# pySTEPS/pysteps

Hardware: AMD Instinct MI355X
Metric: Mpixels*leadsteps/s (LK+semilag) at 4096x4096 fp32 (higher is better)
Workload: dtype f32

## Files before the change

pysteps_amd/csrc/common.h:

```cpp
#pragma once

#include <hip/hip_runtime.h>

#include <cmath>
#include <cstdarg>
#include <cstddef>
#include <cstdint>
#include <cstdio>
#include <mutex>

#include "../../include/pysteps_hip.h"
#include "entry.h"
#include "scratch.h"

#ifdef PSH_DEBUG
#include <cassert>
#define PSH_DASSERT(cond) assert(cond)
#else
#define PSH_DASSERT(cond) ((void)0)
#endif

namespace psh {

constexpr int kNumXcd = 8;
// ... 128 lines not shown
                                  int capacity, int k, double thr, unsigned char *flags_dev,
                                  hipStream_t stream);
int lk_track_pool(void *pyramid_handle, const float *points_host, const float *points_dev, const int *npts_dev,
                  int npts, int max_count, double epsilon, double min_eig_threshold, double *pool_xy_dev,
                  double *pool_uv_dev, int *pool_count_dev, int pool_capacity);

int lk_corners_resident(const unsigned char *feature_u8_dev, const float *clean_dev, float *stats_dev, int m, int n,
                        int block_size, int buffer_mask, double quality_level, double min_distance, int max_corners,
                        float *points_dev, int *npoints_dev, int (*before_walk)(void *) = nullptr,
                        void *before_walk_arg = nullptr, int *walk_stats_host = nullptr,
                        unsigned *slots_cleared = nullptr);

size_t lk_prepare_ws_bytes(int m, int n, bool f64);
int lk_prepare_on(hipStream_t stream, void *ws, const void *frame_dev, bool f64, int m, int n, int size_opening,
                  int buffer_mask, float *clean_dev, unsigned char *track_u8_dev, unsigned char *feature_u8_dev,
                  float *stats_dev, unsigned *slots_cleared = nullptr, unsigned long long *keepbits = nullptr);
size_t lk_keepbits_bytes(int m, int n);
size_t lk_slot_bytes();
int lk_pyramids_on_side(hipStream_t side, void *block, size_t block_bytes, const unsigned char *prev_u8_dev,
                        const unsigned char *next_u8_dev, int m, int n, int win_w, int win_h, int max_level,
                        void **handle_out);
size_t lk_pyramids_bytes(int m, int n, int win_w, int win_h, int max_level);

int corner_order_max_corners();
bool corner_order_supported(int m, int n, double min_distance, int max_corners);
size_t corner_order_ws_bytes();
hipError_t launch_corner_order(const unsigned long long *raw_dev, const int *raw_count_dev, int cap,
                               const float *eig_max_dev, float quality, int n, double min_distance,
                               int max_corners, void *ws_dev, float *points_dev, int *npoints_dev,
                               hipStream_t stream, int (*before_walk)(void *), void *before_walk_arg,
                               bool ws_is_cleared, const unsigned *eig_slots_dev = nullptr, int count_bias = 0,
                               float *eig_max_out_dev = nullptr);
size_t corner_order_clear_bytes();
size_t corner_order_walk_stats_offset();
hipError_t launch_vectors_finish(const double *pool_xy_dev, const double *pool_uv_dev,
                                 const unsigned char *flags_dev, const int *pool_count_dev, int capacity,
                                 double decl_scale, int m, int n, float *xy_out_dev, float *uv_out_dev,
                                 IdwDyn *dyn_dev, hipStream_t stream);

}
```

pysteps_amd/csrc/lk.hip:

```cpp
#include <algorithm>
#include <cmath>
#include <cstring>
#include <functional>
#include <vector>

#include "common.h"

#pragma clang fp contract(off)

namespace psh {
namespace {

enum Stat : int {
  kMinAll = 0,
  kNanCount,
  kMaxAll,
  kMinFeat,
  kMaxFeat,
  kEigMax,
  kNumStats = 8
};

constexpr int kRedBlocks = 1024;

// ... 619 lines not shown
  return true;
}

__device__ __forceinline__ float next_lane_f(float v) {
  return __int_as_float(__builtin_amdgcn_update_dpp(0, __float_as_int(v), 0x130 , 0xf, 0xf, true));
}
__device__ __forceinline__ double next_lane_d(double v) {
  const int lo = __builtin_amdgcn_update_dpp(0, __double2loint(v), 0x130, 0xf, 0xf, true);
  const int hi = __builtin_amdgcn_update_dpp(0, __double2hiint(v), 0x130, 0xf, 0xf, true);
  return __hiloint2double(hi, lo);
}
__device__ __forceinline__ bool walk_mirrored(int i, int n) {
  if (i >= 0 && i + 1 < n) return false;
  return reflect101(i + 1, n) != reflect101(reflect101(i, n) + 1, n);
}

constexpr int crn_cols(int block_size) { return 64 - 2 * (block_size / 2 + 1); }

template <int BS, int ROWS>
__global__ __launch_bounds__(256) void lk_corner_response_cols(
    const unsigned char *__restrict__ u8, const float *__restrict__ clean, int m, int n,
    int buffer_mask, const float *__restrict__ stats, float *__restrict__ eig,
    float *__restrict__ partial, Band band, unsigned *__restrict__ slots, int *__restrict__ zero_a, int count_a,
    int *__restrict__ zero_b, int count_b) {
  constexpr int r = BS / 2, H = r + 1, W = crn_cols(BS);
  if (blockIdx.x == 0 && blockIdx.y == 0) {
    for (int i = threadIdx.x; i < count_a; i += 256) zero_a[i] = 0;
    for (int i = threadIdx.x; i < count_b; i += 256) zero_b[i] = 0;
  }
  __shared__ float red[4];
  const int lane = threadIdx.x & 63, wave = __builtin_amdgcn_readfirstlane(threadIdx.x >> 6);
  const int x0 = blockIdx.x * W;
  const int yb = (blockIdx.y * 4 + wave) * ROWS;
  float best = 0.f;
  if (yb < m) {
    const float s = 1.0f / (4.0f * static_cast<float>(BS) * 255.0f), s2 = 2.f * s;
    const int xl = x0 - H + lane;
    const bool neg_x = walk_mirrored(xl + 1, n);
    const float sx = neg_x ? -s : s, sx2 = neg_x ? -s2 : s2;
    const unsigned char *col = u8 + reflect101(xl, n);
    const bool few_rows = m < 2 * H + 2;
    auto row_of = [&](int y) -> int {
      if (few_rows) return reflect101(y, m);
      y = y < 0 ? -y : y;
      return y >= m ? 2 * m - 2 - y : y;
    };
    auto load_row = [&](int i) -> int { return col[static_cast<size_t>(row_of(yb - H + i)) * n]; };
// ... 58 lines not shown
            t1 = next_lane_d(t1);
            t2 = next_lane_d(t2);
            w0 += t0;
            w1 += t1;
            w2 += t2;
          }
          const int y = yb + p - BS;
          if (writer) {
            const float a = static_cast<float>(w0) * 0.5f, b = static_cast<float>(w1);
            const float c = static_cast<float>(w2) * 0.5f;
            const float e = (a + c) - sqrtf((a - c) * (a - c) + b * b);
            eig[static_cast<size_t>(y) * n + x] = e;
            if (y >= band.lo && y < band.hi && px_allowed(clean, m, n, x, y, buffer_mask, any_nan))
              best = fmaxf(best, fmaxf(e, 0.f));
          }
        }
      }
#pragma unroll
      for (int j = 0; j < BS; ++j) raw[j] = nxt[j];
    }
  }
  best = wave_max(best);
  if (lane == 0) red[wave] = best;
  __syncthreads();
  if (threadIdx.x == 0) {
    const int b = blockIdx.y * gridDim.x + blockIdx.x;
    const float b_max = fmaxf(fmaxf(red[0], red[1]), fmaxf(red[2], red[3]));
    if (slots) {
      slot_max(slots, kSlEig, b, b_max);
    } else {
      partial[b] = b_max;
    }
  }
}

constexpr int kNmsKeys = 64;

using CornerKeyT = unsigned long long;
__device__ __forceinline__ CornerKeyT nms_key(float val, unsigned addr) {
  return (static_cast<CornerKeyT>(__float_as_uint(val)) << 32) | addr;
}
__device__ __forceinline__ float prev_lane_f(float v) {
  return __int_as_float(__builtin_amdgcn_update_dpp(0, __float_as_int(v), 0x138 , 0xf, 0xf, true));
}

template <int BS, int ROWS>
// ... 168 lines not shown

#ifndef PSH_SEL_WAVES
#define PSH_SEL_WAVES 4
#endif
#ifndef PSH_SEL_GROUPS
#define PSH_SEL_GROUPS 4
#endif
#ifndef PSH_SEL_WIDE
#define PSH_SEL_WIDE 1
#endif
constexpr int kSelWaves = PSH_SEL_WAVES;
constexpr int kSelGroups = PSH_SEL_GROUPS;
constexpr bool kSelWide = PSH_SEL_WIDE != 0;
constexpr int kSelCols = 62;
constexpr int kSelWgRows = kSelWide ? 16 * kSelGroups : 16 * kSelGroups * kSelWaves;
constexpr int kSelWgCols = kSelWide ? kSelCols * kSelWaves : kSelCols;

__global__ __launch_bounds__(64 * kSelWaves) void lk_corner_select(const float *__restrict__ eig,
                                                        const float *__restrict__ clean, int m,
                                                        int n, int buffer_mask, float quality,
                                                        float *__restrict__ stats,
                                                        CornerKey *__restrict__ out, int cap,
                                                        int *__restrict__ count, Band band,
                                                        const unsigned *__restrict__ slots) {
  constexpr int kRows = 16;
  __shared__ unsigned long long s_mask[kSelWaves][kSelGroups * kRows];
  __shared__ int wave_count[kSelWaves];
  __shared__ int block_base;
  const int lane = threadIdx.x & 63, wave = threadIdx.x >> 6;
  const int x = (kSelWide ? (blockIdx.x * kSelWaves + wave) : blockIdx.x) * kSelCols - 1 + lane, xc = x + 1;
  const int y_wave = (kSelWide ? blockIdx.y : (blockIdx.y * kSelWaves + wave)) * (kSelGroups * kRows);
  const float eig_max = slots ? slots_max(slots, kSlEig) : stats[kEigMax];
  if (slots && blockIdx.x == 0 && blockIdx.y == 0 && threadIdx.x == 0) stats[kEigMax] = eig_max;
  const float thr = eig_max * quality;
  const bool any_nan = stats[kNanCount] > 0.f;
  const bool col_in = x >= 0 && x < n;
  const bool col_ok = lane < kSelCols && xc >= 1 && xc < n - 1;
  int mine = 0;
  for (int g = 0; g < kSelGroups; ++g) {
    const int y_first = y_wave + g * kRows;
    if (y_first >= m) {
      if (lane < kRows) s_mask[wave][g * kRows + lane] = 0ull;
      continue;
    }
    float v[kRows + 2], m3[kRows + 2], hmax[kRows + 2];
#pragma unroll
    for (int q = 0; q < kRows + 2; ++q) {
      const int y = y_first - 1 + q;
      v[q] = (col_in && y >= 0 && y < m) ? eig[static_cast<size_t>(y) * n + x] : 0.f;
    }
#pragma unroll
    for (int q = 0; q < kRows + 2; ++q) {
      const float left = v[q], centre = next_lane_f(left), right = next_lane_f(centre);
      hmax[q] = fmaxf(left, right);
      m3[q] = fmaxf(centre, hmax[q]);
      v[q] = centre;
    }
#pragma unroll
    for (int r = 0; r < kRows; ++r) {
      const int yr = y_first + r;
      const float c = v[r + 1];
      bool keep = col_ok && yr >= 1 && yr < m - 1 && yr >= band.lo && yr < band.hi;
      keep = keep && c > thr && c != 0.f;
      keep = keep && !(fmaxf(hmax[r + 1], fmaxf(m3[r], m3[r + 2])) > c);
      keep = keep && px_allowed(clean, m, n, xc, yr, buffer_mask, any_nan);
      const unsigned long long mask = __ballot(keep);
      if (lane == 0) s_mask[wave][g * kRows + r] = mask;
      mine += __popcll(mask);
    }
  }
  if (lane == 0) wave_count[wave] = mine;
  __syncthreads();
  if (threadIdx.x == 0) {
    int total = 0;
    for (int w = 0; w < kSelWaves; ++w) total += wave_count[w];
    block_base = total > 0 ? atomicAdd(count, total) : 0;
  }
  __syncthreads();
  int pos = block_base;
  for (int w = 0; w < wave; ++w) pos += wave_count[w];
  if (mine == 0) return;
  for (int r = 0; r < kSelGroups * kRows; ++r) {
    const unsigned long long mask = s_mask[wave][r];
    if (mask == 0ull) continue;
    const int y = y_wave + r;
    if ((mask >> lane) & 1ull) {
      const int at = pos + __popcll(mask & ((1ull << lane) - 1ull));
      if (at < cap)
        out[at] = make_corner_key(eig[static_cast<size_t>(y) * n + xc], static_cast<unsigned>(y + band.y_org) * n + xc);
    }
    pos += __popcll(mask);
  }
}

constexpr int kPyrRows = 8;

struct PyrPair {
  const unsigned char *src[2];
  unsigned char *dst[2];
};

template <bool FAST>
__device__ __forceinline__ void pyr_rows(const unsigned char *__restrict__ src, unsigned char *__restrict__ dst, int m,
                                         int n, int om, int on, int ox, int oy0, int wx, const int (&off)[11]) {
  auto window = [&](const unsigned char *row) -> uint4 {
    if (FAST) return *reinterpret_cast<const uint4 *>(row + wx);
    unsigned w[4] = {0u, 0u, 0u, 0u};
#pragma unroll
    for (int k = 0; k < 11; ++k) w[(k + 2) >> 2] |= static_cast<unsigned>(row[off[k]]) << (8 * ((k + 2) & 3));
    return make_uint4(w[0], w[1], w[2], w[3]);
  };
  auto hrow = [&](const uint4 d, int h[4]) {
    const unsigned w[4] = {d.x, d.y, d.z, d.w};
    auto b = [&](int k) -> int { return static_cast<int>((w[(k + 2) >> 2] >> (8 * ((k + 2) & 3))) & 0xffu); };
// ... 564 lines not shown
  return dim3((n + w - 1) / w, (m + rows - 1) / rows);
}
int lk_response_nms_fixed_keys(dim3 grid) { return static_cast<int>(grid.x * grid.y) * 4 * kNmsKeys; }
void launch_lk_response_nms(dim3 grid, hipStream_t stream, int block_size, const unsigned char *u8, const float *clean, int m,
                            int n, int buffer_mask, const float *stats, float quality, CornerKeyT *out, int cap, Band band,
                            unsigned *slots, int *zero_b, int count_b) {
#define PSH_NMS_LAUNCH(BS)                                                                                             \
  hipLaunchKernelGGL((lk_corner_response_nms<BS, kCrnRows>), grid, dim3(256), 0, stream, u8, clean, m, n, buffer_mask, \
                     stats, quality, out, cap, band, slots, zero_b, count_b)
  if (block_size == 1) {
    PSH_NMS_LAUNCH(1);
  } else if (block_size == 3) {
    PSH_NMS_LAUNCH(3);
  } else if (block_size == 5) {
    PSH_NMS_LAUNCH(5);
  } else {
    PSH_NMS_LAUNCH(7);
  }
#undef PSH_NMS_LAUNCH
}
void launch_lk_response(dim3 grid, hipStream_t stream, int block_size, const unsigned char *u8, const float *clean, int m,
                        int n, int buffer_mask, const float *stats, float *eig, float *part, Band band,
                        unsigned *slots = nullptr, int *zero_a = nullptr, int count_a = 0, int *zero_b = nullptr,
                        int count_b = 0) {
#define PSH_CRN_LAUNCH(BS)                                                                                          \
  hipLaunchKernelGGL((lk_corner_response_cols<BS, kCrnRows>), grid, dim3(256), 0, stream, u8, clean, m, n, buffer_mask, \
                     stats, eig, part, band, slots, zero_a, count_a, zero_b, count_b)
  if (block_size == 1) {
    PSH_CRN_LAUNCH(1);
  } else if (block_size == 3) {
    PSH_CRN_LAUNCH(3);
  } else if (block_size == 5) {
    PSH_CRN_LAUNCH(5);
  } else {
    PSH_CRN_LAUNCH(7);
  }
#undef PSH_CRN_LAUNCH
}

static int ensure_lk_ws(size_t nbytes, void **ptr) {
  static void *ws = nullptr;
  const int rc = persistent_device(&ws, nbytes);
  *ptr = ws;
  return rc;
}

size_t lk_prepare_ws_bytes(int m, int n, bool f64) {
  const size_t npx = static_cast<size_t>(m) * n;
  if (f64) {
    const dim3 ogrid((n + kOpenColsW - 1) / kOpenColsW, (m + kOpenRowsWG - 1) / kOpenRowsWG);
// ... 133 lines not shown
  const float *img = frame_dev + static_cast<size_t>(e0) * n;
  float *clean = clean_dev + static_cast<size_t>(e0) * n;
  const psh::Band band{e0, r0 - e0, r1 - e0};
  psh::launch_lk_open(ogrid, c.stream, img, ms, n, size_opening, buffer_mask, stats_dev, clean, part, band);
  hipLaunchKernelGGL(psh::lk_open_final, dim3(1), dim3(psh::kFinalThreads), 0, c.stream, part, nb_open, stats_dev);
  PSH_HIP(hipGetLastError());
  return PSH_OK;
}

int psh_lk_band_to_u8_dev(const float *clean_dev, int m, int n, int e0, int e1, int buffer_mask, const float *stats_dev,
                          unsigned char *track_u8_dev, unsigned char *feature_u8_dev) {
  PSH_ENTER(c);
  if (!clean_dev || !stats_dev || !track_u8_dev) return fail(PSH_EINVAL, "lk_band_to_u8: NULL pointer");
  if (int rc = check_band("lk_band_to_u8", m, n, e0, e1, e0, e1)) return rc;
  const size_t off = static_cast<size_t>(e0) * n, npx = static_cast<size_t>(e1 - e0) * n;
  const int qgrid = static_cast<int>(std::min<size_t>((npx / 4 + 255) / 256 + 1, 4096));
  hipLaunchKernelGGL(psh::lk_to_u8, dim3(qgrid), dim3(256), 0, c.stream, clean_dev + off, e1 - e0, n, buffer_mask,
                     const_cast<float *>(stats_dev), track_u8_dev + off, feature_u8_dev ? feature_u8_dev + off : nullptr, e0,
                     static_cast<const unsigned *>(nullptr));
  PSH_HIP(hipGetLastError());
  return PSH_OK;
}

int psh_lk_band_response_dev(const unsigned char *feature_u8_dev, const float *clean_dev, int m, int n, int e0, int e1,
                             int r0, int r1, int block_size, int buffer_mask, float *stats_dev, float *eig_dev) {
  PSH_ENTER(c);
  if (!feature_u8_dev || !clean_dev || !stats_dev || !eig_dev) return fail(PSH_EINVAL, "lk_band_response: NULL pointer");
  if (int rc = check_band("lk_band_response", m, n, e0, e1, r0, r1)) return rc;
  if (block_size < 1 || block_size > 2 * psh::kMaxBlockR + 1 || (block_size & 1) == 0)
    return fail(PSH_EUNSUPPORTED, "lk_corners: block_size %d not implemented (odd, <= 7)", block_size);
  const int ms = e1 - e0;
  const dim3 rgrid = psh::lk_response_grid(ms, n, block_size);
  const int nb = rgrid.x * rgrid.y;
  void *ws = nullptr;
  if (int rc = psh::ensure_lk_ws(sizeof(float) * static_cast<size_t>(nb), &ws)) return rc;
  float *part = static_cast<float *>(ws);
  const size_t off = static_cast<size_t>(e0) * n;
  const psh::Band band{e0, r0 - e0, r1 - e0};
  psh::launch_lk_response(rgrid, c.stream, block_size, feature_u8_dev + off, clean_dev + off, ms, n, buffer_mask, stats_dev,
                          eig_dev + off, part, band);
  hipLaunchKernelGGL(psh::lk_max_final, dim3(1), dim3(psh::kFinalThreads), 0, c.stream, part, nb, stats_dev,
                     static_cast<int>(psh::kEigMax), static_cast<int *>(nullptr), 0, static_cast<int *>(nullptr), 0);
  PSH_HIP(hipGetLastError());
  return PSH_OK;
}

int psh_lk_band_select_dev(const float *eig_dev, const float *clean_dev, int m, int n, int e0, int e1, int r0, int r1,
                           int buffer_mask, double quality_level, const float *stats_dev,
                           unsigned long long *keys_dev, int cap, int *count_dev) {
  PSH_ENTER(c);
  if (!eig_dev || !clean_dev || !stats_dev || !keys_dev || !count_dev || cap <= 0)
    return fail(PSH_EINVAL, "lk_band_select: invalid argument");
  if (int rc = check_band("lk_band_select", m, n, e0, e1, r0, r1)) return rc;
  const int ms = e1 - e0;
  const size_t off = static_cast<size_t>(e0) * n;
  PSH_HIP(hipMemsetAsync(count_dev, 0, sizeof(int), c.stream));
  PSH_HIP(hipMemsetAsync(keys_dev, 0, static_cast<size_t>(cap) * sizeof(psh::CornerKey), c.stream));
  const dim3 sgrid((n + psh::kSelWgCols - 1) / psh::kSelWgCols, (ms + psh::kSelWgRows - 1) / psh::kSelWgRows);
  hipLaunchKernelGGL(psh::lk_corner_select, sgrid, dim3(64 * psh::kSelWaves), 0, c.stream, eig_dev + off, clean_dev + off, ms, n,
                     buffer_mask, static_cast<float>(quality_level), const_cast<float *>(stats_dev), keys_dev, cap, count_dev,
                     psh::Band{e0, r0 - e0, r1 - e0}, static_cast<const unsigned *>(nullptr));
  PSH_HIP(hipGetLastError());
  return PSH_OK;
}

namespace {
struct CornerJob {
  bool active = false;
  bool host_ordered = false;
  int m = 0, n = 0, cap = 0, max_corners = 0;
  double min_distance = 0.0;
  psh::CornerKey *raw_dev = nullptr;
  hipEvent_t ready = nullptr;
  void *pinned = nullptr;
  void *ws = nullptr;
};
constexpr size_t kPinnedHeader = 64;
constexpr int kMaxCornerJobs = 4;
CornerJob g_corner_jobs[kMaxCornerJobs];
int g_corner_head = 0, g_corner_count = 0;

struct GreedyGrid {
  int cell, gw, gh, n;
  double md2;
// ... 29 lines not shown
          if (dx * dx + dy * dy < md2) return false;
        }
    const int id = static_cast<int>(px.size());
    px.push_back(x);
    py.push_back(y);
    const int cidx = yc * gw + xc;
    if (head[cidx] < 0) touched.push_back(cidx);
    next.push_back(head[cidx]);
    head[cidx] = id;
    return true;
  }
};
}

namespace {
static int g_lk_fused_nms = [] {
  const char *e = std::getenv("PYSTEPS_HIP_LK_FUSED_NMS");
  return e ? std::atoi(e) : 0;
}();
}
extern "C++" {
namespace psh {
void set_lk_fused_nms(int v) { g_lk_fused_nms = v; }
}
}
namespace {
struct CornerWs {
  size_t off_part, off_cnt, off_raw, off_ord, bytes;
  int cap, nb;
  dim3 rgrid;
  CornerWs(int m, int n, int block_size) {
    const size_t npx = static_cast<size_t>(m) * n;
    rgrid = psh::lk_response_grid(m, n, block_size);
    nb = rgrid.x * rgrid.y;
    cap = static_cast<int>(std::min<size_t>(npx, 0x7fffffffu));
    cap = std::max(cap, psh::lk_response_nms_fixed_keys(psh::lk_response_nms_grid(m, n, block_size)));
    auto up = [](size_t v) { return (v + 255) & ~static_cast<size_t>(255); };
    off_part = up(npx * sizeof(float));
    off_cnt = up(off_part + static_cast<size_t>(nb) * sizeof(float));
    off_raw = up(off_cnt + sizeof(int));
    off_ord = up(off_raw + static_cast<size_t>(cap) * sizeof(psh::CornerKey));
    bytes = off_ord + psh::corner_order_ws_bytes();
  }
};

int corner_candidates(const CornerWs &w, void *ws, const unsigned char *feature_u8_dev, const float *clean_dev,
                      float *stats_dev, int m, int n, int block_size, int buffer_mask, double quality_level,
                      unsigned *eig_slots = nullptr, const int **count_dev_out = nullptr, int *count_bias_out = nullptr) {
  psh::Context &c = ctx();
  char *base = static_cast<char *>(ws);
  float *eig = reinterpret_cast<float *>(base);
  float *part = reinterpret_cast<float *>(base + w.off_part);
  int *cnt = reinterpret_cast<int *>(base + w.off_cnt);
  psh::CornerKey *raw = reinterpret_cast<psh::CornerKey *>(base + w.off_raw);
  int *ord = reinterpret_cast<int *>(base + w.off_ord);
  const int ord_ints = static_cast<int>(psh::corner_order_clear_bytes() / sizeof(int));
  if (count_dev_out) *count_dev_out = cnt;
  if (eig_slots && count_dev_out && count_bias_out && g_lk_fused_nms) {
    const dim3 ngrid = psh::lk_response_nms_grid(m, n, block_size);
    psh::launch_lk_response_nms(ngrid, c.stream, block_size, feature_u8_dev, clean_dev, m, n, buffer_mask, stats_dev,
                                static_cast<float>(quality_level), raw, w.cap, psh::Band{0, 0, m}, eig_slots, ord, ord_ints);
    *count_dev_out = reinterpret_cast<const int *>(eig_slots + psh::kSlCand * psh::kSlots);
    *count_bias_out = psh::lk_response_nms_fixed_keys(ngrid);
    PSH_HIP(hipGetLastError());
    return PSH_OK;
  }
  if (eig_slots) {
    psh::launch_lk_response(w.rgrid, c.stream, block_size, feature_u8_dev, clean_dev, m, n, buffer_mask, stats_dev, eig,
                            part, psh::Band{0, 0, m}, eig_slots, cnt, 1, ord, ord_ints);
  } else {
    psh::launch_lk_response(w.rgrid, c.stream, block_size, feature_u8_dev, clean_dev, m, n, buffer_mask, stats_dev, eig,
                            part, psh::Band{0, 0, m});
    hipLaunchKernelGGL(psh::lk_max_final, dim3(1), dim3(psh::kFinalThreads), 0, c.stream, part, w.nb, stats_dev,
                       static_cast<int>(psh::kEigMax), cnt, 1, ord, ord_ints);
  }
  const dim3 sgrid((n + psh::kSelWgCols - 1) / psh::kSelWgCols, (m + psh::kSelWgRows - 1) / psh::kSelWgRows);
  hipLaunchKernelGGL(psh::lk_corner_select, sgrid, dim3(64 * psh::kSelWaves), 0, c.stream, eig, clean_dev, m, n, buffer_mask,
                     static_cast<float>(quality_level), stats_dev, raw, w.cap, cnt, psh::Band{0, 0, m},
                     static_cast<const unsigned *>(eig_slots));
  PSH_HIP(hipGetLastError());
  return PSH_OK;
}

int check_corner_args(const unsigned char *feature_u8_dev, const float *clean_dev, const float *stats_dev, int m,
                      int n, int block_size, int max_corners) {
  if (m <= 0 || n <= 0) return fail(PSH_EINVAL, "lk_corners: invalid shape (%d,%d)", m, n);
  if (!feature_u8_dev || !clean_dev || !stats_dev) return fail(PSH_EINVAL, "lk_corners: NULL pointer");
  if (block_size < 1 || block_size > 2 * psh::kMaxBlockR + 1 || (block_size & 1) == 0)
    return fail(PSH_EUNSUPPORTED, "lk_corners: block_size %d not implemented (odd, <= 7)", block_size);
  if (max_corners <= 0) return fail(PSH_EINVAL, "lk_corners: max_corners must be positive");
  if (static_cast<uint64_t>(m) * static_cast<uint64_t>(n) >= (1ull << 31))
    return fail(PSH_EUNSUPPORTED, "lk_corners: more than 2^31 pixels");
  return PSH_OK;
}
}

extern "C++" {
namespace psh {
int lk_corners_resident(const unsigned char *feature_u8_dev, const float *clean_dev, float *stats_dev, int m, int n,
                        int block_size, int buffer_mask, double quality_level, double min_distance, int max_corners,
                        float *points_dev, int *npoints_dev, int (*before_walk)(void *), void *before_walk_arg,
                        int *walk_stats_host, unsigned *slots_cleared) {
  if (int rc = check_corner_args(feature_u8_dev, clean_dev, stats_dev, m, n, block_size, max_corners)) return rc;
  if (!points_dev || !npoints_dev) return fail(PSH_EINVAL, "lk_corners: NULL pointer");
  if (!corner_order_supported(m, n, min_distance, max_corners))
    return fail(PSH_EUNSUPPORTED, "lk_corners: more than %d corners or 65535 rows / columns are ordered on the host",
                corner_order_max_corners());
  Context &c = ctx();
  const CornerWs w(m, n, block_size);
  Scratch ws;
  if (int rc = ws.alloc(w.bytes)) return rc;
  const int *count_dev = nullptr;
  int count_bias = 0;
  int rc = corner_candidates(w, ws.as<void>(), feature_u8_dev, clean_dev, stats_dev, m, n, block_size, buffer_mask, quality_level,
                             slots_cleared, &count_dev, &count_bias);
  if (rc == PSH_OK) {
    char *base = ws.as<char>();
    const hipError_t e = launch_corner_order(
        reinterpret_cast<const CornerKey *>(base + w.off_raw), count_dev, w.cap,
        stats_dev + kEigMax, static_cast<float>(quality_level), n, min_distance, max_corners, base + w.off_ord,
        points_dev, npoints_dev, c.stream, before_walk, before_walk_arg, true,
        count_bias ? slots_cleared + psh::kSlEig * psh::kSlots : nullptr, count_bias, count_bias ? stats_dev + kEigMax : nullptr);
    if (e != hipSuccess) rc = fail(PSH_EHIP, "corner_order launch failed: %s", hipGetErrorString(e));
    if (rc == PSH_OK && walk_stats_host) {
      if (hipMemcpyAsync(walk_stats_host, base + w.off_ord + corner_order_walk_stats_offset(), 13 * sizeof(int),
                         hipMemcpyDeviceToHost, c.stream) != hipSuccess ||
          hipStreamSynchronize(c.stream) != hipSuccess)
        rc = fail(PSH_EHIP, "corner_order statistics copy failed");
    }
  }
  return rc;
}
}
}

int psh_lk_corners_launch_dev(const unsigned char *feature_u8_dev, const float *clean_dev,
                              float *stats_dev, int m, int n, int block_size, int buffer_mask,
                              double quality_level, double min_distance, int max_corners) {
  PSH_ENTER(c);
  if (int rc = check_corner_args(feature_u8_dev, clean_dev, stats_dev, m, n, block_size, max_corners)) return rc;
  if (g_corner_count == kMaxCornerJobs)
    return fail(PSH_EINVAL, "lk_corners: %d corner requests are already in flight", kMaxCornerJobs);
  CornerJob &job = g_corner_jobs[(g_corner_head + g_corner_count) % kMaxCornerJobs];
  if (!job.ready) PSH_HIP(hipEventCreateWithFlags(&job.ready, hipEventDisableTiming));
  const bool host_ordered = !psh::corner_order_supported(m, n, min_distance, max_corners);
// ... 97 lines not shown
namespace psh {
[[maybe_unused]] static const int g_corner_jobs_hook = at_shutdown([] {
  for (CornerJob &job : g_corner_jobs) {
    if (job.ready) (void)hipEventDestroy(job.ready);
    job = CornerJob{};
  }
  g_corner_head = g_corner_count = 0;
});
int lk_corners_in_flight_limit() { return kMaxCornerJobs; }
}
}

int psh_lk_corners_dev(const unsigned char *feature_u8_dev, const float *clean_dev,
                       float *stats_dev, int m, int n, int block_size, int buffer_mask,
                       double quality_level, double min_distance, int max_corners,
                       float *points_host, int *count_host) {
  if (!points_host || !count_host) return fail(PSH_EINVAL, "lk_corners: NULL pointer");
  if (int rc = psh_lk_corners_launch_dev(feature_u8_dev, clean_dev, stats_dev, m, n, block_size,
                                         buffer_mask, quality_level, min_distance, max_corners))
    return rc;
  return psh_lk_corners_finish(points_host, count_host);
}

namespace {
struct PyramidSet {
  psh::Pyramid pyr;
  void *block = nullptr;
  hipStream_t stream = nullptr;
  int win_w = 0, win_h = 0, max_level = 0;
};
}

static int lk_pyramids_on(hipStream_t stream, const unsigned char *prev_u8_dev, const unsigned char *next_u8_dev,
                          int m, int n, int win_w, int win_h, int max_level, void **handle_out, void *block_in,
                          size_t block_in_bytes);

int psh_lk_pyramids_dev(const unsigned char *prev_u8_dev, const unsigned char *next_u8_dev, int m,
                        int n, int win_w, int win_h, int max_level, void **handle_out) {
  PSH_ENTER(c);
  return lk_pyramids_on(c.stream, prev_u8_dev, next_u8_dev, m, n, win_w, win_h, max_level, handle_out, nullptr, 0);
}

extern "C++" {
namespace psh {
int lk_pyramids_on_side(hipStream_t side, void *block, size_t block_bytes, const unsigned char *prev_u8_dev,
                        const unsigned char *next_u8_dev, int m, int n, int win_w, int win_h, int max_level,
// ... 315 lines not shown
```

pysteps_amd/csrc/lk_sparse.hip:

```cpp
#include <cstddef>

#include "common.h"

namespace psh {
namespace {

using CornerKey = unsigned long long;

constexpr int kOrdThreads = 1024;
constexpr int kOrdWaves = kOrdThreads / 64;
constexpr int kOrdBins = 1024;
constexpr int kChunkCap = 4096;
constexpr int kMaxCornersDev = 2048;
constexpr int kHashSlots = 8192;

template <bool DESC>
__device__ __forceinline__ void bitonic_sort_lds(unsigned long long *keys, int p2) {
  for (int k = 2; k <= p2; k <<= 1) {
    for (int j = k >> 1; j > 0; j >>= 1) {
      for (int t = threadIdx.x; t < (p2 >> 1); t += blockDim.x) {
        const int i = ((t & ~(j - 1)) << 1) | (t & (j - 1)), o = i | j;
        const unsigned long long a = keys[i], b = keys[o];
        const bool first_half = (i & k) == 0;
        if ((first_half == DESC) ? a < b : a > b) {
          keys[i] = b;
          keys[o] = a;
        }
      }
      const int next_j = j > 1 ? (j >> 1) : k;
      if (j > 64 || next_j > 64 || (k == p2 && j == 1)) {
        __syncthreads();
      } else {
        __builtin_amdgcn_fence(__ATOMIC_RELEASE, "wavefront");
        __builtin_amdgcn_wave_barrier();
        __builtin_amdgcn_fence(__ATOMIC_ACQUIRE, "wavefront");
      }
    }
  }
}

__device__ __forceinline__ int next_pow2(int v) {
  int p = 128;
  while (p < v) p <<= 1;
  return p;
}

__device__ __forceinline__ void key_range(float eig_max, float quality, CornerKey &key_lo, CornerKey &key_hi) {
  const float top = fmaxf(eig_max, 0.f);
  const float thr = fmaxf(top * quality, 0.f);
  key_lo = (static_cast<CornerKey>(__float_as_uint(thr)) + 1ull) << 32;
  key_hi = (static_cast<CornerKey>(__float_as_uint(top)) + 1ull) << 32;
}
__device__ __forceinline__ float load_eig_max(const float *eig_max, const unsigned *eig_slots) {
  if (eig_slots == nullptr) return *eig_max;
  unsigned v = eig_slots[threadIdx.x & 63];
#pragma unroll
  for (int d = 32; d >= 1; d >>= 1) {
    const unsigned o = static_cast<unsigned>(__shfl_xor(static_cast<int>(v), d));
    v = o > v ? o : v;
  }
  return __uint_as_float((v >> 31) ? (v & 0x7fffffffu) : ~v);
}
__device__ __forceinline__ int bin_shift(CornerKey rlo, CornerKey rhi) {
  int sh = 0;
  while (((rhi - 1ull - rlo) >> sh) >= static_cast<unsigned long long>(kOrdBins)) ++sh;
  return sh;
}

__device__ __forceinline__ void chunk_cut(const int *hist, int above, int lane, int ccap, int &over_out, int &fits_out) {
  constexpr int kPer = kOrdBins / 64;
  int tot = 0;
  for (int q = 0; q < kPer; ++q) tot += hist[lane * kPer + q];
  int incl = tot;
#pragma unroll
  for (int d = 1; d < 64; d <<= 1) {
    const int dn = __shfl_down(incl, d);
    if (lane + d < 64) incl += dn;
  }
  int run = incl - tot + above;
  int over = -1, over_next = 0;
  for (int q = kPer - 1; q >= 0; --q) {
    const int before = run;
    run += hist[lane * kPer + q];
    if (run > ccap && over < 0) {
      over = lane * kPer + q;
      over_next = before;
    }
  }
  int best = over;
#pragma unroll
  for (int d = 32; d >= 1; d >>= 1) best = max(best, __shfl_xor(best, d));
// ... 744 lines not shown
}

}

int corner_order_max_corners() { return kMaxCornersDev; }

constexpr size_t kOrdOffHdr = kOrdBins * sizeof(int);
constexpr size_t kOrdOffHead = kOrdOffHdr + 128;
static_assert(sizeof(OrderHeader) <= 128, "header slot");
static_assert(offsetof(OrderHeader, phase_us) == offsetof(OrderHeader, walk) + 3 * sizeof(int), "walk statistics are one int[13]");
size_t corner_order_ws_bytes() { return kOrdOffHead + static_cast<size_t>(kHeadSegs) * kChunkCap * sizeof(CornerKey); }

size_t corner_order_clear_bytes() { return kOrdOffHead; }
size_t corner_order_walk_stats_offset() { return kOrdOffHdr + offsetof(OrderHeader, walk); }

bool corner_order_supported(int m, int n, double min_distance, int max_corners) {
  return max_corners <= kMaxCornersDev && m <= 65535 && n <= 65535 && min_distance < 16383.0;
}

hipError_t launch_corner_order(const unsigned long long *raw_dev, const int *raw_count_dev, int cap,
                               const float *eig_max_dev, float quality, int n, double min_distance,
                               int max_corners, void *ws_dev, float *points_dev, int *npoints_dev,
                               hipStream_t stream, int (*before_walk)(void *), void *before_walk_arg,
                               bool ws_is_cleared, const unsigned *eig_slots_dev, int count_bias, float *eig_max_out_dev) {
  const int cell = static_cast<int>(std::lrint(min_distance)) > 1 ? static_cast<int>(std::lrint(min_distance)) : 1;
  const double md2 = std::ceil(min_distance * min_distance);
  const unsigned md2_ceil = md2 >= 2147483647.0 ? 2147483647u : static_cast<unsigned>(md2);
  char *ws = static_cast<char *>(ws_dev);
  int *hist = reinterpret_cast<int *>(ws);
  OrderHeader *hdr = reinterpret_cast<OrderHeader *>(ws + kOrdOffHdr);
  CornerKey *head = reinterpret_cast<CornerKey *>(ws + kOrdOffHead);
  if (!ws_is_cleared) {
    const hipError_t e = hipMemsetAsync(ws, 0, kOrdOffHead, stream);
    if (e != hipSuccess) return e;
  }
  const int groups = std::max(1, std::min(128, (cap + 4 * kPreThreads - 1) / (4 * kPreThreads)));
  hipLaunchKernelGGL(corner_hist, dim3(groups), dim3(kPreThreads), 0, stream, raw_dev, raw_count_dev, cap, eig_max_dev,
                     quality, hist, eig_slots_dev, count_bias);
  int ccap = 1024;
  while (ccap < 2 * max_corners && ccap < kChunkCap) ccap <<= 1;
  hipLaunchKernelGGL(corner_gather, dim3(groups), dim3(kPreThreads), 0, stream, raw_dev, raw_count_dev, cap, eig_max_dev,
                     quality, hist, head, hdr, ccap, eig_slots_dev, count_bias);
  if (before_walk != nullptr && before_walk(before_walk_arg) != 0) return hipErrorUnknown;
  hipLaunchKernelGGL(corner_order, dim3(1), dim3(kOrdThreads), 0, stream, raw_dev, raw_count_dev, cap, eig_max_dev,
                     quality, head, hdr, n, cell, md2_ceil, min_distance >= 1.0 ? 1 : 0, max_corners, ccap,
                     reinterpret_cast<float2 *>(points_dev), npoints_dev, eig_slots_dev, count_bias, eig_max_out_dev);
  return hipGetLastError();
}

hipError_t launch_vectors_finish(const double *pool_xy_dev, const double *pool_uv_dev,
                                 const unsigned char *flags_dev, const int *pool_count_dev, int capacity,
                                 double decl_scale, int m, int n, float *xy_out_dev, float *uv_out_dev,
                                 IdwDyn *dyn_dev, hipStream_t stream) {
  hipLaunchKernelGGL(vectors_finish, dim3(1), dim3(kOrdThreads), 0, stream,
                     reinterpret_cast<const double2 *>(pool_xy_dev), reinterpret_cast<const double2 *>(pool_uv_dev),
                     flags_dev, pool_count_dev, capacity, decl_scale, m, n, reinterpret_cast<float2 *>(xy_out_dev),
                     reinterpret_cast<float2 *>(uv_out_dev), dyn_dev);
  return hipGetLastError();
}

}

extern "C" int psh_lk_order_host(const unsigned long long *keys_host, int count, float response_max,
                                 double quality_level, int m, int n, double min_distance, int max_corners,
                                 float *points_host, int *count_host) {
  PSH_ENTER(c);
  if (!points_host || !count_host || (count > 0 && !keys_host)) return psh::fail(PSH_EINVAL, "lk_order: NULL pointer");
  if (count < 0 || m <= 0 || n <= 0 || max_corners <= 0) return psh::fail(PSH_EINVAL, "lk_order: invalid argument");
  if (!psh::corner_order_supported(m, n, min_distance, max_corners))
// ... 79 lines not shown
```

pysteps_amd/csrc/runtime.hip:

```cpp
#include <cmath>
#include <cstdlib>
#include <cstring>
#include <map>
#include <vector>

#include "common.h"
#include "registry.h"

namespace psh {

Context &ctx() {
  static Context c;
  return c;
}

static thread_local char g_err[512] = "";

int fail(int code, const char *fmt, ...) {
  va_list ap;
  va_start(ap, fmt);
  vsnprintf(g_err, sizeof(g_err), fmt, ap);
  va_end(ap);
  return code;
}
// ... 187 lines not shown
  if (std::strcmp(key, "semilag_variant") == 0) {
    if (value != 0 && value != 1 && value != 5 && value != 7 && value != 12)
      return fail(PSH_EINVAL,
                  "semilag_variant must be 0 (window kernel where it applies, gather kernels elsewhere), 12 (window kernel "
                  "for every eligible call), 7 (gather kernels: packed {u,v} plane + row-pair field plane), 5 (packed "
                  "velocity only) or 1 (one plane per component, DPP column sharing)");
    psh::set_semilag_variant(value);
    return PSH_OK;
  }
  if (std::strcmp(key, "members_variant") == 0) {
    if (value != 1 && value != 2)
      return fail(PSH_EINVAL, "members_variant must be 2 (two members per thread, default) or 1 (one)");
    psh::set_members_variant(value);
    return PSH_OK;
  }
  if (std::strcmp(key, "idw_variant") == 0) {
    if (value < 0 || value > 1) return fail(PSH_EINVAL, "idw_variant must be 0 (two-level) or 1 (pre-pass per 16x16 tile)");
    psh::set_idw_variant(value);
    return PSH_OK;
  }
  if (std::strcmp(key, "lk_fused_nms") == 0) {
    if (value != 0 && value != 1) return fail(PSH_EINVAL, "lk_fused_nms must be 0 (response + selection passes, default) or 1 (one fused pass)");
    psh::set_lk_fused_nms(value);
    return PSH_OK;
  }
  if (std::strcmp(key, "trim_cache") == 0) {
    psh::Context &c = ctx();
    psh::Lock lock(c.mu);
    if (c.ready) {
      if (int rc = psh::bind_device(c.device)) return rc;
      PSH_HIP(hipStreamSynchronize(c.stream));
      psh::release_cache();
      psh::pinned_release_cache();
    }
    return PSH_OK;
  }
  return fail(PSH_EINVAL, "psh_set_option: unknown option '%s'", key);
}

int psh_field_stats_dev(const float *in_dev, size_t n, double *min_out, double *max_out,
                        double *nonfinite_out, double *nanmin_out);

int psh_device_info(int *device_id, int *cu_count, size_t *hbm_total, size_t *hbm_free,
                    char *name, int name_len) {
  PSH_ENTER(c);
  if (device_id) *device_id = c.device;
// ... 290 lines not shown
```

Before: 278,800.

## Skip cold tiles in corner selection using per-wave response maxima and fuse histogram

The corner response kernel now writes a per-wave block maximum of the eigenvalue response. The selection pass reads these maxima and skips 16-row groups whose blocks cannot exceed the quality threshold, so it no longer reads the whole response plane. It also builds the corner-order key histogram in shared memory during selection, which lets the separate corner_hist launch be dropped. This adds a small per-block write, extra workspace, host-side bookkeeping for band mode and shared-memory atomics in the selection kernel.

```diff
diff --git a/pysteps_amd/csrc/common.h b/pysteps_amd/csrc/common.h
--- a/pysteps_amd/csrc/common.h
+++ b/pysteps_amd/csrc/common.h
@@ -174,6 +174,20 @@
                         void **handle_out);
 size_t lk_pyramids_bytes(int m, int n, int win_w, int win_h, int max_level);
 
+constexpr int kOrdBins = 1024;
+__device__ __forceinline__ void key_range(float eig_max, float quality, unsigned long long &key_lo,
+                                          unsigned long long &key_hi) {
+  const float top = fmaxf(eig_max, 0.f);
+  const float thr = fmaxf(top * quality, 0.f);
+  key_lo = (static_cast<unsigned long long>(__float_as_uint(thr)) + 1ull) << 32;
+  key_hi = (static_cast<unsigned long long>(__float_as_uint(top)) + 1ull) << 32;
+}
+__device__ __forceinline__ int bin_shift(unsigned long long rlo, unsigned long long rhi) {
+  int sh = 0;
+  while (((rhi - 1ull - rlo) >> sh) >= static_cast<unsigned long long>(kOrdBins)) ++sh;
+  return sh;
+}
+
 int corner_order_max_corners();
 bool corner_order_supported(int m, int n, double min_distance, int max_corners);
 size_t corner_order_ws_bytes();
@@ -182,7 +196,10 @@
                                int max_corners, void *ws_dev, float *points_dev, int *npoints_dev,
                                hipStream_t stream, int (*before_walk)(void *), void *before_walk_arg,
                                bool ws_is_cleared, const unsigned *eig_slots_dev = nullptr, int count_bias = 0,
-                               float *eig_max_out_dev = nullptr);
+                               float *eig_max_out_dev = nullptr, bool hist_is_built = false);
+hipError_t launch_corner_hist(const unsigned long long *raw_dev, const int *raw_count_dev, int cap,
+                              const float *eig_max_dev, float quality, int *hist_dev, hipStream_t stream);
+void set_lk_select_skip(int v);
 size_t corner_order_clear_bytes();
 size_t corner_order_walk_stats_offset();
 hipError_t launch_vectors_finish(const double *pool_xy_dev, const double *pool_uv_dev,
diff --git a/pysteps_amd/csrc/lk.hip b/pysteps_amd/csrc/lk.hip
--- a/pysteps_amd/csrc/lk.hip
+++ b/pysteps_amd/csrc/lk.hip
@@ -665,7 +665,7 @@
     const unsigned char *__restrict__ u8, const float *__restrict__ clean, int m, int n,
     int buffer_mask, const float *__restrict__ stats, float *__restrict__ eig,
     float *__restrict__ partial, Band band, unsigned *__restrict__ slots, int *__restrict__ zero_a, int count_a,
-    int *__restrict__ zero_b, int count_b) {
+    int *__restrict__ zero_b, int count_b, float *__restrict__ blockmax) {
   constexpr int r = BS / 2, H = r + 1, W = crn_cols(BS);
   if (blockIdx.x == 0 && blockIdx.y == 0) {
     for (int i = threadIdx.x; i < count_a; i += 256) zero_a[i] = 0;
@@ -770,6 +770,7 @@
   }
   best = wave_max(best);
   if (lane == 0) red[wave] = best;
+  if (blockmax != nullptr && lane == 0) blockmax[static_cast<size_t>(blockIdx.y * 4 + wave) * gridDim.x + blockIdx.x] = best;
   __syncthreads();
   if (threadIdx.x == 0) {
     const int b = blockIdx.y * gridDim.x + blockIdx.x;
@@ -984,12 +985,15 @@
                                                         float *__restrict__ stats,
                                                         CornerKey *__restrict__ out, int cap,
                                                         int *__restrict__ count, Band band,
-                                                        const unsigned *__restrict__ slots) {
+                                                        const unsigned *__restrict__ slots,
+                                                        const float *__restrict__ blockmax, int bm_pitch, int bm_w,
+                                                        int bm_rows, int *__restrict__ hist) {
   constexpr int kRows = 16;
   __shared__ unsigned long long s_mask[kSelWaves][kSelGroups * kRows];
   __shared__ int wave_count[kSelWaves];
-  __shared__ int block_base;
-  const int lane = threadIdx.x & 63, wave = threadIdx.x >> 6;
+  __shared__ int block_base, block_total;
+  __shared__ int s_hist[kOrdBins];
+  const int lane = threadIdx.x & 63, wave = __builtin_amdgcn_readfirstlane(threadIdx.x >> 6);
   const int x = (kSelWide ? (blockIdx.x * kSelWaves + wave) : blockIdx.x) * kSelCols - 1 + lane, xc = x + 1;
   const int y_wave = (kSelWide ? blockIdx.y : (blockIdx.y * kSelWaves + wave)) * (kSelGroups * kRows);
   const float eig_max = slots ? slots_max(slots, kSlEig) : stats[kEigMax];
@@ -998,10 +1002,28 @@
   const bool any_nan = stats[kNanCount] > 0.f;
   const bool col_in = x >= 0 && x < n;
   const bool col_ok = lane < kSelCols && xc >= 1 && xc < n - 1;
+  unsigned hot = ~0u;
+  if (blockmax != nullptr) {
+    hot = 0u;
+    const float thr_u = __int_as_float(__builtin_amdgcn_readfirstlane(__float_as_int(thr)));
+    const int xj = (kSelWide ? (blockIdx.x * kSelWaves + wave) : blockIdx.x) * kSelCols;
+    if (xj < n) {
+      const int cb0 = xj / bm_w, cb1 = min(xj + kSelCols - 1, n - 1) / bm_w;
+      for (int g = 0; g < kSelGroups; ++g) {
+        const int y_first = y_wave + g * kRows;
+        if (y_first >= m) break;
+        const int rb0 = y_first / bm_rows, rb1 = min(y_first + kRows - 1, m - 1) / bm_rows;
+        bool any = false;
+        for (int rb = rb0; rb <= rb1; ++rb)
+          for (int cb = cb0; cb <= cb1; ++cb) any = any || blockmax[static_cast<size_t>(rb) * bm_pitch + cb] > thr_u;
+        hot |= any ? 1u << g : 0u;
+      }
+    }
+  }
   int mine = 0;
   for (int g = 0; g < kSelGroups; ++g) {
     const int y_first = y_wave + g * kRows;
-    if (y_first >= m) {
+    if (y_first >= m || !((hot >> g) & 1u)) {
       if (lane < kRows) s_mask[wave][g * kRows + lane] = 0ull;
       continue;
     }
@@ -1037,21 +1059,38 @@
     int total = 0;
     for (int w = 0; w < kSelWaves; ++w) total += wave_count[w];
     block_base = total > 0 ? atomicAdd(count, total) : 0;
+    block_total = total;
   }
   __syncthreads();
+  if (block_total == 0) return;
   int pos = block_base;
   for (int w = 0; w < wave; ++w) pos += wave_count[w];
-  if (mine == 0) return;
-  for (int r = 0; r < kSelGroups * kRows; ++r) {
+  CornerKey key_lo = 0ull, key_hi = 0ull;
+  int sh = 0;
+  if (hist != nullptr) {
+    for (int i = threadIdx.x; i < kOrdBins; i += 64 * kSelWaves) s_hist[i] = 0;
+    key_range(eig_max, quality, key_lo, key_hi);
+    sh = bin_shift(key_lo, key_hi);
+    __syncthreads();
+  }
+  for (int r = 0; mine != 0 && r < kSelGroups * kRows; ++r) {
     const unsigned long long mask = s_mask[wave][r];
     if (mask == 0ull) continue;
     const int y = y_wave + r;
     if ((mask >> lane) & 1ull) {
       const int at = pos + __popcll(mask & ((1ull << lane) - 1ull));
-      if (at < cap)
-        out[at] = make_corner_key(eig[static_cast<size_t>(y) * n + xc], static_cast<unsigned>(y + band.y_org) * n + xc);
+      if (at < cap) {
+        const CornerKey k = make_corner_key(eig[static_cast<size_t>(y) * n + xc], static_cast<unsigned>(y + band.y_org) * n + xc);
+        out[at] = k;
+        if (hist != nullptr && k >= key_lo && k < key_hi) atomicAdd(&s_hist[static_cast<int>((k - key_lo) >> sh)], 1);
+      }
     }
     pos += __popcll(mask);
+  }
+  if (hist != nullptr) {
+    __syncthreads();
+    for (int i = threadIdx.x; i < kOrdBins; i += 64 * kSelWaves)
+      if (s_hist[i]) atomicAdd(&hist[i], s_hist[i]);
   }
 }
 
@@ -1662,10 +1701,10 @@
 void launch_lk_response(dim3 grid, hipStream_t stream, int block_size, const unsigned char *u8, const float *clean, int m,
                         int n, int buffer_mask, const float *stats, float *eig, float *part, Band band,
                         unsigned *slots = nullptr, int *zero_a = nullptr, int count_a = 0, int *zero_b = nullptr,
-                        int count_b = 0) {
+                        int count_b = 0, float *blockmax = nullptr) {
 #define PSH_CRN_LAUNCH(BS)                                                                                          \
   hipLaunchKernelGGL((lk_corner_response_cols<BS, kCrnRows>), grid, dim3(256), 0, stream, u8, clean, m, n, buffer_mask, \
-                     stats, eig, part, band, slots, zero_a, count_a, zero_b, count_b)
+                     stats, eig, part, band, slots, zero_a, count_a, zero_b, count_b, blockmax)
   if (block_size == 1) {
     PSH_CRN_LAUNCH(1);
   } else if (block_size == 3) {
@@ -1845,6 +1884,33 @@
   return PSH_OK;
 }
 
+namespace {
+int lk_select_skip_default() {
+  const char *e = std::getenv("PYSTEPS_HIP_LK_SELECT_SKIP");
+  return e ? std::atoi(e) : 1;
+}
+int g_lk_select_skip = lk_select_skip_default();
+
+struct BandMax {
+  const float *eig = nullptr, *clean = nullptr, *stats = nullptr;
+  int n = 0, e0 = 0, e1 = 0, r0 = 0, r1 = 0, buffer_mask = 0, w = 0, pitch = 0;
+  float *dev = nullptr;
+};
+constexpr int kBandMaxSlots = 4;
+BandMax g_band_max[kBandMaxSlots];
+int g_band_max_next = 0;
+BandMax *band_max_find(const float *eig) {
+  for (BandMax &b : g_band_max)
+    if (b.eig == eig && b.dev != nullptr) return &b;
+  return nullptr;
+}
+void band_max_forget() {
+  for (BandMax &b : g_band_max) b.eig = nullptr;
+  g_band_max_next = 0;
+}
+[[maybe_unused]] const int g_band_max_hook = psh::at_shutdown(band_max_forget);
+}
+
 int psh_lk_band_response_dev(const unsigned char *feature_u8_dev, const float *clean_dev, int m, int n, int e0, int e1,
                              int r0, int r1, int block_size, int buffer_mask, float *stats_dev, float *eig_dev) {
   PSH_ENTER(c);
@@ -1860,8 +1926,18 @@
   float *part = static_cast<float *>(ws);
   const size_t off = static_cast<size_t>(e0) * n;
   const psh::Band band{e0, r0 - e0, r1 - e0};
+  BandMax *bm = band_max_find(eig_dev);
+  if (bm) bm->eig = nullptr;
+  if (g_lk_select_skip) {
+    if (!bm) bm = &g_band_max[g_band_max_next++ % kBandMaxSlots];
+    bm->eig = nullptr;
+    if (int rc = psh::persistent_device(reinterpret_cast<void **>(&bm->dev), static_cast<size_t>(nb) * 4 * sizeof(float))) return rc;
+    *bm = BandMax{eig_dev, clean_dev, stats_dev, n, e0, e1, r0, r1, buffer_mask, psh::crn_cols(block_size), static_cast<int>(rgrid.x), bm->dev};
+  } else {
+    bm = nullptr;
+  }
   psh::launch_lk_response(rgrid, c.stream, block_size, feature_u8_dev + off, clean_dev + off, ms, n, buffer_mask, stats_dev,
-                          eig_dev + off, part, band);
+                          eig_dev + off, part, band, nullptr, nullptr, 0, nullptr, 0, bm ? bm->dev : nullptr);
   hipLaunchKernelGGL(psh::lk_max_final, dim3(1), dim3(psh::kFinalThreads), 0, c.stream, part, nb, stats_dev,
                      static_cast<int>(psh::kEigMax), static_cast<int *>(nullptr), 0, static_cast<int *>(nullptr), 0);
   PSH_HIP(hipGetLastError());
@@ -1880,9 +1956,16 @@
   PSH_HIP(hipMemsetAsync(count_dev, 0, sizeof(int), c.stream));
   PSH_HIP(hipMemsetAsync(keys_dev, 0, static_cast<size_t>(cap) * sizeof(psh::CornerKey), c.stream));
   const dim3 sgrid((n + psh::kSelWgCols - 1) / psh::kSelWgCols, (ms + psh::kSelWgRows - 1) / psh::kSelWgRows);
+  BandMax *bm = g_lk_select_skip ? band_max_find(eig_dev) : nullptr;
+  if (bm && !(bm->clean == clean_dev && bm->stats == stats_dev && bm->n == n && bm->e0 == e0 && bm->e1 == e1 && bm->r0 == r0 && bm->r1 == r1 &&
+              bm->buffer_mask == buffer_mask))
+    bm = nullptr;
+  if (bm) bm->eig = nullptr;
   hipLaunchKernelGGL(psh::lk_corner_select, sgrid, dim3(64 * psh::kSelWaves), 0, c.stream, eig_dev + off, clean_dev + off, ms, n,
                      buffer_mask, static_cast<float>(quality_level), const_cast<float *>(stats_dev), keys_dev, cap, count_dev,
-                     psh::Band{e0, r0 - e0, r1 - e0}, static_cast<const unsigned *>(nullptr));
+                     psh::Band{e0, r0 - e0, r1 - e0}, static_cast<const unsigned *>(nullptr),
+                     static_cast<const float *>(bm ? bm->dev : nullptr), bm ? bm->pitch : 0, bm ? bm->w : 1, psh::kCrnRows,
+                     static_cast<int *>(nullptr));
   PSH_HIP(hipGetLastError());
   return PSH_OK;
 }
@@ -1958,11 +2041,12 @@
 extern "C++" {
 namespace psh {
 void set_lk_fused_nms(int v) { g_lk_fused_nms = v; }
+void set_lk_select_skip(int v) { g_lk_select_skip = v; }
 }
 }
 namespace {
 struct CornerWs {
-  size_t off_part, off_cnt, off_raw, off_ord, bytes;
+  size_t off_part, off_bmax, off_cnt, off_raw, off_ord, bytes;
   int cap, nb;
   dim3 rgrid;
   CornerWs(int m, int n, int block_size) {
@@ -1973,7 +2057,8 @@
     cap = std::max(cap, psh::lk_response_nms_fixed_keys(psh::lk_response_nms_grid(m, n, block_size)));
     auto up = [](size_t v) { return (v + 255) & ~static_cast<size_t>(255); };
     off_part = up(npx * sizeof(float));
-    off_cnt = up(off_part + static_cast<size_t>(nb) * sizeof(float));
+    off_bmax = up(off_part + static_cast<size_t>(nb) * sizeof(float));
+    off_cnt = up(off_bmax + static_cast<size_t>(nb) * 4 * sizeof(float));
     off_raw = up(off_cnt + sizeof(int));
     off_ord = up(off_raw + static_cast<size_t>(cap) * sizeof(psh::CornerKey));
     bytes = off_ord + psh::corner_order_ws_bytes();
@@ -1982,11 +2067,14 @@
 
 int corner_candidates(const CornerWs &w, void *ws, const unsigned char *feature_u8_dev, const float *clean_dev,
                       float *stats_dev, int m, int n, int block_size, int buffer_mask, double quality_level,
-                      unsigned *eig_slots = nullptr, const int **count_dev_out = nullptr, int *count_bias_out = nullptr) {
+                      unsigned *eig_slots = nullptr, const int **count_dev_out = nullptr, int *count_bias_out = nullptr,
+                      bool *hist_built_out = nullptr) {
   psh::Context &c = ctx();
   char *base = static_cast<char *>(ws);
   float *eig = reinterpret_cast<float *>(base);
   float *part = reinterpret_cast<float *>(base + w.off_part);
+  float *bmax = g_lk_select_skip ? reinterpret_cast<float *>(base + w.off_bmax) : nullptr;
+  if (hist_built_out) *hist_built_out = false;
   int *cnt = reinterpret_cast<int *>(base + w.off_cnt);
   psh::CornerKey *raw = reinterpret_cast<psh::CornerKey *>(base + w.off_raw);
   int *ord = reinterpret_cast<int *>(base + w.off_ord);
@@ -2003,17 +2091,19 @@
   }
   if (eig_slots) {
     psh::launch_lk_response(w.rgrid, c.stream, block_size, feature_u8_dev, clean_dev, m, n, buffer_mask, stats_dev, eig,
-                            part, psh::Band{0, 0, m}, eig_slots, cnt, 1, ord, ord_ints);
+                            part, psh::Band{0, 0, m}, eig_slots, cnt, 1, ord, ord_ints, bmax);
   } else {
     psh::launch_lk_response(w.rgrid, c.stream, block_size, feature_u8_dev, clean_dev, m, n, buffer_mask, stats_dev, eig,
-                            part, psh::Band{0, 0, m});
+                            part, psh::Band{0, 0, m}, nullptr, nullptr, 0, nullptr, 0, bmax);
     hipLaunchKernelGGL(psh::lk_max_final, dim3(1), dim3(psh::kFinalThreads), 0, c.stream, part, w.nb, stats_dev,
                        static_cast<int>(psh::kEigMax), cnt, 1, ord, ord_ints);
   }
   const dim3 sgrid((n + psh::kSelWgCols - 1) / psh::kSelWgCols, (m + psh::kSelWgRows - 1) / psh::kSelWgRows);
   hipLaunchKernelGGL(psh::lk_corner_select, sgrid, dim3(64 * psh::kSelWaves), 0, c.stream, eig, clean_dev, m, n, buffer_mask,
                      static_cast<float>(quality_level), stats_dev, raw, w.cap, cnt, psh::Band{0, 0, m},
-                     static_cast<const unsigned *>(eig_slots));
+                     static_cast<const unsigned *>(eig_slots), static_cast<const float *>(bmax), static_cast<int>(w.rgrid.x),
+                     psh::crn_cols(block_size), psh::kCrnRows, (bmax && hist_built_out) ? ord : static_cast<int *>(nullptr));
+  if (hist_built_out) *hist_built_out = bmax != nullptr;
   PSH_HIP(hipGetLastError());
   return PSH_OK;
 }
@@ -2048,15 +2138,17 @@
   if (int rc = ws.alloc(w.bytes)) return rc;
   const int *count_dev = nullptr;
   int count_bias = 0;
+  bool hist_built = false;
   int rc = corner_candidates(w, ws.as<void>(), feature_u8_dev, clean_dev, stats_dev, m, n, block_size, buffer_mask, quality_level,
-                             slots_cleared, &count_dev, &count_bias);
+                             slots_cleared, &count_dev, &count_bias, &hist_built);
   if (rc == PSH_OK) {
     char *base = ws.as<char>();
     const hipError_t e = launch_corner_order(
         reinterpret_cast<const CornerKey *>(base + w.off_raw), count_dev, w.cap,
         stats_dev + kEigMax, static_cast<float>(quality_level), n, min_distance, max_corners, base + w.off_ord,
         points_dev, npoints_dev, c.stream, before_walk, before_walk_arg, true,
-        count_bias ? slots_cleared + psh::kSlEig * psh::kSlots : nullptr, count_bias, count_bias ? stats_dev + kEigMax : nullptr);
+        count_bias ? slots_cleared + psh::kSlEig * psh::kSlots : nullptr, count_bias, count_bias ? stats_dev + kEigMax : nullptr,
+        hist_built);
     if (e != hipSuccess) rc = fail(PSH_EHIP, "corner_order launch failed: %s", hipGetErrorString(e));
     if (rc == PSH_OK && walk_stats_host) {
       if (hipMemcpyAsync(walk_stats_host, base + w.off_ord + corner_order_walk_stats_offset(), 13 * sizeof(int),
@@ -2200,6 +2292,35 @@
   return psh_lk_corners_finish(points_host, count_host);
 }
 
+int psh_lk_select_probe_dev(const unsigned char *feature_u8_dev, const float *clean_dev, float *stats_dev, int m, int n,
+                            int block_size, int buffer_mask, double quality_level, int cap, unsigned long long *keys_dev,
+                            int *count_dev, int *hist_dev, int *hist_ref_dev) {
+  PSH_ENTER(c);
+  if (int rc = check_corner_args(feature_u8_dev, clean_dev, stats_dev, m, n, block_size, 1)) return rc;
+  if (!keys_dev || !count_dev || !hist_dev || !hist_ref_dev || cap <= 0) return fail(PSH_EINVAL, "lk_select_probe: invalid argument");
+  CornerWs w(m, n, block_size);
+  w.cap = std::min(w.cap, cap);
+  psh::Scratch ws;
+  if (int rc = ws.alloc(w.bytes)) return rc;
+  bool hist_built = false;
+  if (int rc = corner_candidates(w, ws.as<void>(), feature_u8_dev, clean_dev, stats_dev, m, n, block_size, buffer_mask,
+                                 quality_level, nullptr, nullptr, nullptr, &hist_built))
+    return rc;
+  const psh::CornerKey *raw = ws.at<psh::CornerKey>(w.off_raw);
+  const int *cnt = ws.at<int>(w.off_cnt);
+  int *ord = ws.at<int>(w.off_ord);
+  const float quality = static_cast<float>(quality_level);
+  if (!hist_built) PSH_HIP(psh::launch_corner_hist(raw, cnt, w.cap, stats_dev + psh::kEigMax, quality, ord, c.stream));
+  PSH_HIP(hipMemsetAsync(keys_dev, 0, static_cast<size_t>(cap) * sizeof(psh::CornerKey), c.stream));
+  PSH_HIP(hipMemcpyAsync(keys_dev, raw, static_cast<size_t>(w.cap) * sizeof(psh::CornerKey), hipMemcpyDeviceToDevice, c.stream));
+  PSH_HIP(hipMemcpyAsync(count_dev, cnt, sizeof(int), hipMemcpyDeviceToDevice, c.stream));
+  PSH_HIP(hipMemcpyAsync(hist_dev, ord, psh::kOrdBins * sizeof(int), hipMemcpyDeviceToDevice, c.stream));
+  PSH_HIP(hipMemsetAsync(hist_ref_dev, 0, psh::kOrdBins * sizeof(int), c.stream));
+  PSH_HIP(psh::launch_corner_hist(raw, cnt, w.cap, stats_dev + psh::kEigMax, quality, hist_ref_dev, c.stream));
+  PSH_HIP(hipStreamSynchronize(c.stream));
+  return PSH_OK;
+}
+
 namespace {
 struct PyramidSet {
   psh::Pyramid pyr;
diff --git a/pysteps_amd/csrc/lk_sparse.hip b/pysteps_amd/csrc/lk_sparse.hip
--- a/pysteps_amd/csrc/lk_sparse.hip
+++ b/pysteps_amd/csrc/lk_sparse.hip
@@ -9,7 +9,6 @@
 
 constexpr int kOrdThreads = 1024;
 constexpr int kOrdWaves = kOrdThreads / 64;
-constexpr int kOrdBins = 1024;
 constexpr int kChunkCap = 4096;
 constexpr int kMaxCornersDev = 2048;
 constexpr int kHashSlots = 8192;
@@ -45,12 +44,6 @@
   return p;
 }
 
-__device__ __forceinline__ void key_range(float eig_max, float quality, CornerKey &key_lo, CornerKey &key_hi) {
-  const float top = fmaxf(eig_max, 0.f);
-  const float thr = fmaxf(top * quality, 0.f);
-  key_lo = (static_cast<CornerKey>(__float_as_uint(thr)) + 1ull) << 32;
-  key_hi = (static_cast<CornerKey>(__float_as_uint(top)) + 1ull) << 32;
-}
 __device__ __forceinline__ float load_eig_max(const float *eig_max, const unsigned *eig_slots) {
   if (eig_slots == nullptr) return *eig_max;
   unsigned v = eig_slots[threadIdx.x & 63];
@@ -61,12 +54,6 @@
   }
   return __uint_as_float((v >> 31) ? (v & 0x7fffffffu) : ~v);
 }
-__device__ __forceinline__ int bin_shift(CornerKey rlo, CornerKey rhi) {
-  int sh = 0;
-  while (((rhi - 1ull - rlo) >> sh) >= static_cast<unsigned long long>(kOrdBins)) ++sh;
-  return sh;
-}
-
 __device__ __forceinline__ void chunk_cut(const int *hist, int above, int lane, int ccap, int &over_out, int &fits_out) {
   constexpr int kPer = kOrdBins / 64;
   int tot = 0;
@@ -857,7 +844,8 @@
                                const float *eig_max_dev, float quality, int n, double min_distance,
                                int max_corners, void *ws_dev, float *points_dev, int *npoints_dev,
                                hipStream_t stream, int (*before_walk)(void *), void *before_walk_arg,
-                               bool ws_is_cleared, const unsigned *eig_slots_dev, int count_bias, float *eig_max_out_dev) {
+                               bool ws_is_cleared, const unsigned *eig_slots_dev, int count_bias, float *eig_max_out_dev,
+                               bool hist_is_built) {
   const int cell = static_cast<int>(std::lrint(min_distance)) > 1 ? static_cast<int>(std::lrint(min_distance)) : 1;
   const double md2 = std::ceil(min_distance * min_distance);
   const unsigned md2_ceil = md2 >= 2147483647.0 ? 2147483647u : static_cast<unsigned>(md2);
@@ -865,13 +853,15 @@
   int *hist = reinterpret_cast<int *>(ws);
   OrderHeader *hdr = reinterpret_cast<OrderHeader *>(ws + kOrdOffHdr);
   CornerKey *head = reinterpret_cast<CornerKey *>(ws + kOrdOffHead);
+  if (hist_is_built && !ws_is_cleared) return hipErrorInvalidValue;
   if (!ws_is_cleared) {
     const hipError_t e = hipMemsetAsync(ws, 0, kOrdOffHead, stream);
     if (e != hipSuccess) return e;
   }
   const int groups = std::max(1, std::min(128, (cap + 4 * kPreThreads - 1) / (4 * kPreThreads)));
-  hipLaunchKernelGGL(corner_hist, dim3(groups), dim3(kPreThreads), 0, stream, raw_dev, raw_count_dev, cap, eig_max_dev,
-                     quality, hist, eig_slots_dev, count_bias);
+  if (!hist_is_built)
+    hipLaunchKernelGGL(corner_hist, dim3(groups), dim3(kPreThreads), 0, stream, raw_dev, raw_count_dev, cap, eig_max_dev,
+                       quality, hist, eig_slots_dev, count_bias);
   int ccap = 1024;
   while (ccap < 2 * max_corners && ccap < kChunkCap) ccap <<= 1;
   hipLaunchKernelGGL(corner_gather, dim3(groups), dim3(kPreThreads), 0, stream, raw_dev, raw_count_dev, cap, eig_max_dev,
@@ -880,6 +870,14 @@
   hipLaunchKernelGGL(corner_order, dim3(1), dim3(kOrdThreads), 0, stream, raw_dev, raw_count_dev, cap, eig_max_dev,
                      quality, head, hdr, n, cell, md2_ceil, min_distance >= 1.0 ? 1 : 0, max_corners, ccap,
                      reinterpret_cast<float2 *>(points_dev), npoints_dev, eig_slots_dev, count_bias, eig_max_out_dev);
+  return hipGetLastError();
+}
+
+hipError_t launch_corner_hist(const unsigned long long *raw_dev, const int *raw_count_dev, int cap,
+                              const float *eig_max_dev, float quality, int *hist_dev, hipStream_t stream) {
+  const int groups = std::max(1, std::min(128, (cap + 4 * kPreThreads - 1) / (4 * kPreThreads)));
+  hipLaunchKernelGGL(corner_hist, dim3(groups), dim3(kPreThreads), 0, stream, raw_dev, raw_count_dev, cap, eig_max_dev,
+                     quality, hist_dev, static_cast<const unsigned *>(nullptr), 0);
   return hipGetLastError();
 }
 
diff --git a/pysteps_amd/csrc/runtime.hip b/pysteps_amd/csrc/runtime.hip
--- a/pysteps_amd/csrc/runtime.hip
+++ b/pysteps_amd/csrc/runtime.hip
@@ -233,6 +233,13 @@
   if (std::strcmp(key, "lk_fused_nms") == 0) {
     if (value != 0 && value != 1) return fail(PSH_EINVAL, "lk_fused_nms must be 0 (response + selection passes, default) or 1 (one fused pass)");
     psh::set_lk_fused_nms(value);
+    return PSH_OK;
+  }
+  if (std::strcmp(key, "lk_select_skip") == 0) {
+    if (value != 0 && value != 1)
+      return fail(PSH_EINVAL, "lk_select_skip must be 1 (the selection pass skips blocks below the threshold and bins its keys, "
+                              "default) or 0 (it reads the whole response plane, corner_hist bins)");
+    psh::set_lk_select_skip(value);
     return PSH_OK;
   }
   if (std::strcmp(key, "trim_cache") == 0) {
```

Measured after the change: 278,200 (median of 2 runs). Within noise of the previous version (-0.2%).
